# lenke182/flood-uav-video-segmentation

Hardware: AMD Instinct MI355X
Metric: segmentation FPS @713x713 (PSPNet-ResNet50 keyframe + linear interp, frame_delta=5) (higher is better)
Workload: dtype f32

## Files before the change

flood_uav_video_segmentation_amd/csrc/flow_ops.hip:

```cpp
#include "interp.h"
#include "kernels.h"

#include <type_traits>

namespace fs {

#define FS_LAUNCH_INDEXED(kernel_, total_, cap_, s_, ...)                                                                  \
    do {                                                                                                                   \
        const dim3 grid_((unsigned)std::min<int64_t>(cdiv64((total_), 256), (cap_)));                                      \
        if ((total_) < ((int64_t)1 << 31)) hipLaunchKernelGGL((kernel_<unsigned>), grid_, dim3(256), 0, (s_), __VA_ARGS__); \
        else hipLaunchKernelGGL((kernel_<int64_t>), grid_, dim3(256), 0, (s_), __VA_ARGS__);                               \
    } while (0)

template <typename I>
__global__ __launch_bounds__(256) void grid_sample_nchw_kernel(const float* __restrict__ in, int B, int C, int Hi, int Wi,
                                                               const float* __restrict__ grid, int Hg, int Wg,
                                                               float* __restrict__ out, int ac) {
    const I total = (I)B * Hg * Wg;
    for (I i = (I)blockIdx.x * 256 + threadIdx.x; i < total; i += (I)gridDim.x * 256) {
        const int b = (int)(i / ((I)Hg * Wg));
        const I g = i - (I)b * Hg * Wg;
        const float gx = grid[i * 2 + 0], gy = grid[i * 2 + 1];
        const GsTaps t = gs_taps(gx, gy, Wi, Hi, ac);
        for (int c = 0; c < C; ++c) {
// ... 46 lines not shown
        const int oy = (int)((i / Wo) % Ho);
        const I pc = i / ((I)Wo * Ho);
        const LinCoord cy = lin_coord(oy, Hi, sy, ac), cx = lin_coord(ox, Wi, sx, ac);
        out[i] = bilerp_at(in + (size_t)pc * Hi * Wi, Wi, cy, cx);
    }
}

int launch_resize_bilinear_nchw(const float* in, int BC, int Hi, int Wi, float* out, int Ho, int Wo, int align_corners,
                                hipStream_t s) {
    const int64_t total = (int64_t)BC * Ho * Wo;
    FS_LAUNCH_INDEXED(resize_bilinear_nchw_kernel, total, 16384, s, in, BC, Hi, Wi, out, Ho, Wo, align_corners,
                      resize_scale(Hi, Ho, align_corners), resize_scale(Wi, Wo, align_corners));
    FS_HIP(hipGetLastError());
    return 0;
}

template <typename I>
__global__ __launch_bounds__(256) void resize_bilinear_nhwc_kernel(const float* __restrict__ in, int ld_in, int B, int C4, int Hi,
                                                                   int Wi, float* __restrict__ out, int ld_out, int Ho, int Wo,
                                                                   int ac, float sy, float sx) {
    const I total = (I)B * Ho * Wo * C4;
    for (I i = (I)blockIdx.x * 256 + threadIdx.x; i < total; i += (I)gridDim.x * 256) {
        const int c4 = (int)(i % C4);
        const I m = i / C4;
        const int ox = (int)(m % Wo);
        const int oy = (int)((m / Wo) % Ho);
        const int b = (int)(m / ((I)Wo * Ho));
        const LinCoord cy = lin_coord(oy, Hi, sy, ac), cx = lin_coord(ox, Wi, sx, ac);
        const float* base = in + (size_t)b * Hi * Wi * ld_in + c4 * 4;
        *reinterpret_cast<f32x4*>(out + (size_t)m * ld_out + c4 * 4) = bilerp4_nhwc(base, Wi, ld_in, cy, cx);
    }
}

int launch_resize_bilinear_nhwc(const float* in, int ld_in, int B, int C, int Hi, int Wi, float* out, int ld_out, int Ho, int Wo,
                                int align_corners, hipStream_t s, int max_blocks) {
    FS_REQUIRE(C % 4 == 0 && ld_in % 4 == 0 && ld_out % 4 == 0, "resize_nhwc: C/ld must be multiples of 4");
    const int64_t total = (int64_t)B * Ho * Wo * (C / 4);
    FS_LAUNCH_INDEXED(resize_bilinear_nhwc_kernel, total, max_blocks, s, in, ld_in, B, C / 4, Hi, Wi, out, ld_out, Ho, Wo, align_corners,
                      resize_scale(Hi, Ho, align_corners), resize_scale(Wi, Wo, align_corners));
    FS_HIP(hipGetLastError());
    return 0;
}

__global__ __launch_bounds__(256) void blend_kernel(const float* __restrict__ a, float wa, const float* __restrict__ b, float wb,
                                                    float* __restrict__ out, int64_t n4, int64_t numel) {
    for (int64_t i = (int64_t)blockIdx.x * 256 + threadIdx.x; i < n4; i += (int64_t)gridDim.x * 256) {
        const f32x4 x = reinterpret_cast<const f32x4*>(a)[i];
        f32x4 r;
        if (b) {
            const f32x4 y = reinterpret_cast<const f32x4*>(b)[i];
#pragma unroll
            for (int e = 0; e < 4; ++e) r[e] = __fadd_rn(__fmul_rn(wa, x[e]), __fmul_rn(wb, y[e]));
        } else {
#pragma unroll
            for (int e = 0; e < 4; ++e) r[e] = __fmul_rn(wa, x[e]);
        }
        reinterpret_cast<f32x4*>(out)[i] = r;
    }
    if (blockIdx.x == 0) {
        for (int64_t i = n4 * 4 + threadIdx.x; i < numel; i += 256)
            out[i] = b ? __fadd_rn(__fmul_rn(wa, a[i]), __fmul_rn(wb, b[i])) : __fmul_rn(wa, a[i]);
    }
}

__global__ __launch_bounds__(256) void blend_scalar_kernel(const float* __restrict__ a, float wa, const float* __restrict__ b, float wb,
                                                           float* __restrict__ out, int64_t numel) {
    for (int64_t i = (int64_t)blockIdx.x * 256 + threadIdx.x; i < numel; i += (int64_t)gridDim.x * 256)
        out[i] = b ? __fadd_rn(__fmul_rn(wa, a[i]), __fmul_rn(wb, b[i])) : __fmul_rn(wa, a[i]);
}

int launch_blend(const float* a, float wa, const float* b, float wb, float* out, int64_t numel, hipStream_t s) {
    if ((((uintptr_t)a | (uintptr_t)b | (uintptr_t)out) & 15) != 0) {
        hipLaunchKernelGGL(blend_scalar_kernel, dim3((unsigned)std::max<int64_t>(1, std::min<int64_t>(cdiv64(numel, 256), 16384))),
                           dim3(256), 0, s, a, wa, b, wb, out, numel);
        FS_HIP(hipGetLastError());
        return 0;
    }
    const int64_t n4 = numel / 4;
    hipLaunchKernelGGL(blend_kernel, dim3((unsigned)std::max<int64_t>(1, std::min<int64_t>(cdiv64(n4, 256), 16384))), dim3(256), 0, s,
                       a, wa, b, wb, out, n4, numel);
    FS_HIP(hipGetLastError());
    return 0;
}

__device__ __forceinline__ float up_at(const float* __restrict__ pl, int h, int w, int y, int x, float sy, float sx) {
    return bilerp_at(pl, w, lin_coord(y, h, sy, 1), lin_coord(x, w, sx, 1));
}

__device__ __forceinline__ void seg_warp_step(const float* lo, const float* src, const float* grid, float* dst, int K, int h, int w, int H,
                                              int W, int Hg, int Wg, int first, float sy, float sx) {
    const int G = Hg * Wg;
    for (int g = blockIdx.x * 256 + threadIdx.x; g < G; g += gridDim.x * 256) {
        const float gx = grid[g * 2 + 0], gy = grid[g * 2 + 1];
        const int Hs = first ? H : Hg, Ws = first ? W : Wg;
        const GsTaps t = gs_taps(gx, gy, Ws, Hs, 0);
        for (int k = 0; k < K; ++k) {
            float v;
            if (first) {
                const float* pl = lo + (size_t)k * h * w;
                v = gs_sample(t, [&](int y, int x) { return up_at(pl, h, w, y, x, sy, sx); });
            } else {
                const float* pl = src + (size_t)k * G;
                v = gs_sample(t, [&](int y, int x) { return pl[y * Ws + x]; });
            }
            dst[(size_t)k * G + g] = v;
        }
    }
}

__global__ __launch_bounds__(256) void seg_warp_step_kernel(const float* __restrict__ lo_prev, const float* __restrict__ lo_next,
                                                            const float* __restrict__ src_f, const float* __restrict__ src_b,
                                                            const float* __restrict__ grid_f, const float* __restrict__ grid_b,
                                                            float* __restrict__ dst_f, float* __restrict__ dst_b, int K, int h,
                                                            int w, int H, int W, int Hg, int Wg, int first, float sy, float sx) {
    const int dir = blockIdx.y;
    seg_warp_step(dir ? lo_next : lo_prev, dir ? src_b : src_f, dir ? grid_b : grid_f, dir ? dst_b : dst_f, K, h, w, H, W, Hg, Wg, first, sy, sx);
}

template <int KMAX, bool WARP, bool CANVAS, bool DEVW>
__global__ __launch_bounds__(256) void seg_fuse_kernel(std::conditional_t<DEVW, SegTailParams, SegFuseArgs> p, float sy_lo, float sx_lo,
                                                       float sy_g, float sx_g) {
    const float* weights = nullptr;
    if constexpr (DEVW) weights = p.weights;
    const int64_t HW = (int64_t)p.H * p.W;
    const int K = p.K, n = p.n;
    const size_t cHW = (size_t)p.cH * p.cW;
    for (int y = blockIdx.y; y < p.H; y += gridDim.y) {
        const int x = blockIdx.x * 256 + threadIdx.x;
        if (x >= p.W) break;
        const int64_t i = (int64_t)y * p.W + x;
        const unsigned off4 = (unsigned)i * 4u;
        const size_t cpix = (size_t)(p.y0 + y) * p.cW + (p.x0 + x);
        float a[KMAX], b[KMAX], v[KMAX];
        auto emit = [&](int f) {
            if (p.out_logits)
#pragma unroll
                for (int k = 0; k < KMAX; ++k)
                    if (k < K) *reinterpret_cast<float*>(reinterpret_cast<char*>(p.out_logits + ((size_t)f * K + k) * HW) + off4) = v[k];
            if (p.out_mask) {
                float best = -INFINITY;
                int arg = 0;
#pragma unroll
                for (int k = 0; k < KMAX; ++k)
                    if (k < K && v[k] > best) { best = v[k]; arg = k; }
                p.out_mask[(size_t)f * HW + i] = (uint8_t)arg;
            }
            if (CANVAS) {
                softmax_k<KMAX>(v, K, [&](int k, float q) { p.canvas[((size_t)f * K + k) * cHW + cpix] += (double)q; });
                if (f == 0) p.count[cpix] += 1.0;
            }
        };
        {
            const LinCoord cy = lin_coord(y, p.h, sy_lo, 1), cx = lin_coord(x, p.w, sx_lo, 1);
#pragma unroll
            for (int k = 0; k < KMAX; ++k) {
                if (k < K) {
                    const float* pl = p.lo_prev + (size_t)k * p.h * p.w;
                    a[k] = bilerp_at(pl, p.w, cy, cx);
                    if (p.lo_next && !WARP) {
                        const float* pn = p.lo_next + (size_t)k * p.h * p.w;
                        b[k] = bilerp_at(pn, p.w, cy, cx);
                    }
                    v[k] = a[k];
                }
            }
            emit(0);
        }
        if (!p.lo_next) continue;
        LinCoord gy_c, gx_c;
        if (WARP) {
            gy_c = lin_coord(y, p.Hg, sy_g, 1);
            gx_c = lin_coord(x, p.Wg, sx_g, 1);
        }
        const int G = p.Hg * p.Wg;
        for (int f = 1; f < n; ++f) {
            const float wa = DEVW ? weights[2 * f] : (float)((double)(n - f) / (double)n);
            const float wb = DEVW ? weights[2 * f + 1] : (float)((double)f / (double)n);
            const bool hold_a = DEVW && wb == 0.f, hold_b = DEVW && !hold_a && wa == 0.f;
#pragma unroll
            for (int k = 0; k < KMAX; ++k) {
                if (k < K) {
                    float va, vb;
                    if (!WARP) {
                        va = a[k];
                        vb = b[k];
                    } else {
                        const float* pf = p.scratch + ((size_t)(f - 1) * K + k) * G;
                        const float* pb = p.scratch + ((size_t)(n - 1) * K + (size_t)(n - f - 1) * K + k) * G;
                        if (!hold_b) va = bilerp_at(pf, p.Wg, gy_c, gx_c);
                        if (!hold_a) vb = bilerp_at(pb, p.Wg, gy_c, gx_c);
                    }
                    v[k] = hold_a ? va : hold_b ? vb : __fadd_rn(__fmul_rn(wa, va), __fmul_rn(wb, vb));
                }
            }
            emit(f);
        }
    }
}

int launch_seg_tail(const SegTailParams& p, hipStream_t s) {
    FS_REQUIRE(p.K >= 1 && p.K <= 32, "seg_tail: K=%d out of range (1..32)", p.K);
    FS_REQUIRE(p.n >= 1, "seg_tail: n must be >= 1");
    FS_REQUIRE(p.out_logits || p.out_mask || p.canvas, "seg_tail: no output requested");
    FS_REQUIRE((int64_t)p.H * p.W < ((int64_t)1 << 30), "seg_tail: frames of at most 2^30 pixels");
    FS_REQUIRE(!p.canvas || (p.count && p.y0 >= 0 && p.x0 >= 0 && p.y0 + p.H <= p.cH && p.x0 + p.W <= p.cW), "seg_tail: crop outside the canvas");
    const float sy_lo = resize_scale(p.h, p.H, 1), sx_lo = resize_scale(p.w, p.W, 1);
    float sy_g = 0.f, sx_g = 0.f;
    const bool warp = p.lo_next && !p.no_warp && p.n > 1;
    if (warp) {
        FS_REQUIRE(p.scratch && p.grids_left && p.grids_right, "seg_tail: warp mode needs grids and scratch");
        sy_g = resize_scale(p.Hg, p.H, 1);
        sx_g = resize_scale(p.Wg, p.W, 1);
        const int G = p.Hg * p.Wg;
        const size_t map = (size_t)p.K * G;
        float* fwd = p.scratch;
        float* bwd = p.scratch + (size_t)(p.n - 1) * map;
        for (int j = 0; j < p.n - 1; ++j) {
            hipLaunchKernelGGL(seg_warp_step_kernel, dim3(cdiv(G, 256), 2), dim3(256), 0, s, p.lo_prev, p.lo_next,
                               j ? fwd + (size_t)(j - 1) * map : nullptr, j ? bwd + (size_t)(j - 1) * map : nullptr,
                               p.grids_left[j], p.grids_right[j], fwd + (size_t)j * map, bwd + (size_t)j * map, p.K, p.h, p.w,
                               p.H, p.W, p.Hg, p.Wg, j == 0 ? 1 : 0, sy_lo, sx_lo);
        }
    }
    const dim3 grid((unsigned)cdiv(p.W, 256), (unsigned)std::min(p.H, 65535)), block(256);
    const bool canvas = p.canvas != nullptr;
    const SegFuseArgs& a = p;
#define FS_SEG_FUSE(KM_, W_, C_)                                                                                                   \
    do {                                                                                                                           \
        if (p.weights) hipLaunchKernelGGL((seg_fuse_kernel<KM_, W_, C_, true>), grid, block, 0, s, p, sy_lo, sx_lo, sy_g, sx_g);    \
        else hipLaunchKernelGGL((seg_fuse_kernel<KM_, W_, C_, false>), grid, block, 0, s, a, sy_lo, sx_lo, sy_g, sx_g);            \
    } while (0)
    if (p.K <= 8) {
        if (warp) { if (canvas) FS_SEG_FUSE(8, true, true); else FS_SEG_FUSE(8, true, false); }
        else { if (canvas) FS_SEG_FUSE(8, false, true); else FS_SEG_FUSE(8, false, false); }
    } else {
        if (warp) { if (canvas) FS_SEG_FUSE(32, true, true); else FS_SEG_FUSE(32, true, false); }
        else { if (canvas) FS_SEG_FUSE(32, false, true); else FS_SEG_FUSE(32, false, false); }
    }
#undef FS_SEG_FUSE
    FS_HIP(hipGetLastError());
    return 0;
}

__global__ __launch_bounds__(256) void feat_warp_step_kernel(const float* __restrict__ src_f, const float* __restrict__ src_b, int Hs, int Ws,
                                                             const float* __restrict__ grid_f, const float* __restrict__ grid_b,
                                                             float* __restrict__ dst_f, float* __restrict__ dst_b, int C4, unsigned total, int S) {
    const int dir = blockIdx.y;
    const float* __restrict__ src = dir ? src_b : src_f;
    const float* __restrict__ grid = dir ? grid_b : grid_f;
    float* __restrict__ dst = dir ? dst_b : dst_f;
    const int ld = C4 * 4;
    const unsigned xcd = blockIdx.x & 7u;
    const unsigned e = (blockIdx.x >> 3) * 256u + threadIdx.x;
    const unsigned m = e / (unsigned)S;
    const int c4 = (int)(xcd * (unsigned)S + (e - m * (unsigned)S));
    if (m >= total || c4 >= C4) return;
    const float gx = grid[m * 2 + 0], gy = grid[m * 2 + 1];
    const GsTaps t = gs_taps(gx, gy, Ws, Hs, 0);
    *reinterpret_cast<f32x4*>(dst + (size_t)m * ld + c4 * 4) = gs_gather_nhwc(src + c4 * 4, Ws, ld, t);
}

struct FeatFuseArgs {
    const float* f_prev;
    const float* f_next;
    const float* chains;
    const float* grid0;
    float* stack;
    int C4, fh, fw, Hg, Wg, H0, W0, n;
    int same_g, same_0;
    float sy_g, sx_g, sy_0, sx_0;
};
struct FeatFuseWArgs : FeatFuseArgs {
    const float* weights;
};

constexpr int FEAT_RUN = 10;

struct GsCell {
    unsigned nw, ne, sw, se;
    float wnw, wne, wsw, wse;
    bool all_in;
    bool x1ok, y1ok;
};

__device__ __forceinline__ GsCell feat_cell(const FeatFuseArgs& a, int gy, int gx) {
    const size_t m = (size_t)gy * a.W0 + gx;
    const float2 g = *reinterpret_cast<const float2*>(a.grid0 + m * 2);
    const GsTaps t = gs_taps(g.x, g.y, a.fw, a.fh, 1);
    const unsigned ld = (unsigned)a.C4 * 4u;
    GsCell c;
    c.nw = (unsigned)(t.y0 * a.fw + t.x0) * ld;
    c.ne = (unsigned)(t.y0 * a.fw + t.x1) * ld;
    c.sw = (unsigned)(t.y1 * a.fw + t.x0) * ld;
    c.se = (unsigned)(t.y1 * a.fw + t.x1) * ld;
    c.wnw = t.nw; c.wne = t.ne; c.wsw = t.sw; c.wse = t.se;
    c.x1ok = t.x1ok; c.y1ok = t.y1ok;
    c.all_in = t.x1ok && t.y1ok;
    return c;
}

__device__ __forceinline__ f32x4 feat_cell_value(const float* __restrict__ cbase, const GsCell& c) {
    const f32x4 vnw = *reinterpret_cast<const f32x4*>(cbase + c.nw);
    f32x4 vne = *reinterpret_cast<const f32x4*>(cbase + c.ne);
    f32x4 vsw = *reinterpret_cast<const f32x4*>(cbase + c.sw);
    f32x4 vse = *reinterpret_cast<const f32x4*>(cbase + c.se);
    if (__builtin_amdgcn_ballot_w64(!c.all_in) != 0) {
        const f32x4 z = {0.f, 0.f, 0.f, 0.f};
        vne = c.x1ok ? vne : z;
        vsw = c.y1ok ? vsw : z;
        vse = c.all_in ? vse : z;
    }
    const f32x2 wnw = {c.wnw, c.wnw}, wne = {c.wne, c.wne}, wsw = {c.wsw, c.wsw}, wse = {c.wse, c.wse};
    f32x4 r;
    r.lo = ((vnw.lo * wnw + vne.lo * wne) + vsw.lo * wsw) + vse.lo * wse;
    r.hi = ((vnw.hi * wnw + vne.hi * wne) + vsw.hi * wsw) + vse.hi * wse;
    return r;
}

constexpr int FEAT_KEY_CH = 4;

__global__ __launch_bounds__(256) void feat_fuse_key_kernel(FeatFuseArgs a, unsigned npix, int S, int LP) {
    const int ld = a.C4 * 4;
    const unsigned xcd = blockIdx.x & 7u;
    const unsigned e = (blockIdx.x >> 3) * 256u + threadIdx.x;
    const unsigned m = e / (unsigned)LP;
    const int l = (int)(e - m * (unsigned)LP);
    if (m >= npix) return;
    const int oy = (int)(m / (unsigned)a.fw), ox = (int)(m - (unsigned)oy * (unsigned)a.fw);
    LinCoord cy, cx;
    if (a.same_0) {
        cy.i0 = cy.i1 = oy; cx.i0 = cx.i1 = ox;
        cy.w0 = cx.w0 = 1.f; cy.w1 = cx.w1 = 0.f;
    } else {
        cy = lin_coord(oy, a.H0, a.sy_0, 1);
        cx = lin_coord(ox, a.W0, a.sx_0, 1);
    }
    const GsCell c00 = feat_cell(a, cy.i0, cx.i0);
    GsCell c01 = c00, c10 = c00, c11 = c00;
    if (!a.same_0) {
        c01 = feat_cell(a, cy.i0, cx.i1);
        c10 = feat_cell(a, cy.i1, cx.i0);
        c11 = feat_cell(a, cy.i1, cx.i1);
    }
    const f32x2 wx0 = {cx.w0, cx.w0}, wx1 = {cx.w1, cx.w1}, wy0 = {cy.w0, cy.w0}, wy1 = {cy.w1, cy.w1};
#pragma unroll 1
    for (int k = 0; k < FEAT_KEY_CH; ++k) {
        const int cc = l + k * LP;
        const int c4 = (int)xcd * S + cc;
        if (cc >= S || c4 >= a.C4) break;
        const float* cbase = a.f_prev + c4 * 4;
        f32x4 r;
        if (a.same_0) {
            r = feat_cell_value(cbase, c00);
        } else {
            const f32x4 v00 = feat_cell_value(cbase, c00), v01 = feat_cell_value(cbase, c01);
            const f32x4 v10 = feat_cell_value(cbase, c10), v11 = feat_cell_value(cbase, c11);
            r.lo = wy0 * (wx0 * v00.lo + wx1 * v01.lo) + wy1 * (wx0 * v10.lo + wx1 * v11.lo);
            r.hi = wy0 * (wx0 * v00.hi + wx1 * v01.hi) + wy1 * (wx0 * v10.hi + wx1 * v11.hi);
        }
        *reinterpret_cast<f32x4*>(a.stack + (size_t)m * ld + c4 * 4) = r;
    }
}

template <bool DEVW>
__global__ __launch_bounds__(256, 6) void feat_fuse_warp_kernel(std::conditional_t<DEVW, FeatFuseWArgs, FeatFuseArgs> a, int S, int nruns) {
    const float* weights = nullptr;
    if constexpr (DEVW) weights = a.weights;
    const int ld = a.C4 * 4;
    const size_t map = (size_t)a.fh * a.fw * ld;
    const unsigned bid = blockIdx.x;
    const unsigned xcd = bid & 7u;
    const unsigned e = (bid >> 3) * 256u + threadIdx.x;
    const unsigned item = e / (unsigned)S;
    const int c4 = (int)(xcd * (unsigned)S + (e - item * (unsigned)S));
    const unsigned rowid = item / (unsigned)nruns;
    const int run = (int)(item - rowid * (unsigned)nruns);
    const int p = 1 + (int)(rowid / (unsigned)a.fh);
    const int oy = (int)(rowid - (unsigned)(p - 1) * (unsigned)a.fh);
    if (p >= a.n || c4 >= a.C4) return;
    const float wa = DEVW ? weights[2 * p] : (float)((double)(a.n - p) / (double)a.n);
    const float wb = DEVW ? weights[2 * p + 1] : (float)((double)p / (double)a.n);
    const bool hold_a = DEVW && wb == 0.f, hold_b = DEVW && !hold_a && wa == 0.f;
    const size_t cmap = (size_t)a.Hg * a.Wg * ld;
    const float* pf = a.chains + (size_t)(p - 1) * cmap + c4 * 4;
    const float* pb = a.chains + (size_t)(a.n - 1 + a.n - p - 1) * cmap + c4 * 4;
// ... 625 lines not shown
```

flood_uav_video_segmentation_amd/csrc/net_ops.hip:

```cpp
#include "interp.h"
#include "kernels.h"
#include "split.h"

#include <type_traits>

namespace fs {

template <int CPT >
__global__ __launch_bounds__(256) void stem_conv_kernel(StemParams p) {
    extern __shared__ __attribute__((aligned(16))) float wlds[];
    const int taps = p.KH * p.KW * 3;
    for (int i = threadIdx.x; i < taps * p.Cout; i += 256) wlds[i] = p.wgt[i];
    __syncthreads();

    const int groups = p.Cout / CPT;
    const int ppb = 256 / groups;
    const int cg = threadIdx.x % groups;
    const int M = p.B * p.Ho * p.Wo;
    const int m = blockIdx.x * ppb + threadIdx.x / groups;
    if (m >= M) return;
    const int hw = p.Ho * p.Wo;
    const int b = m / hw;
    const int rem = m - b * hw;
    const int oy = rem / p.Wo, ox = rem - oy * p.Wo;
// ... 256 lines not shown
        if (nsteps <= 2) FS_STEM_SPLIT_PF(NT_, 2) else FS_STEM_SPLIT_PF(NT_, 5)                                                  \
    }
        switch (p.Cout / 32) {
            case 1: FS_STEM_SPLIT(1) break;
            case 2: FS_STEM_SPLIT(2) break;
            case 3: FS_STEM_SPLIT(3) break;
            default: FS_STEM_SPLIT(4) break;
        }
#undef FS_STEM_SPLIT
#undef FS_STEM_SPLIT_PF
        FS_HIP(hipGetLastError());
        return 0;
    }
    if (p.Cout % 32 == 0 && p.Cout <= 128 && p.KH < 0x7fff) {
        const int ksteps = cdiv(cdiv(taps, 2), 8) * 8;
        const size_t lds = (size_t)2 * ksteps * (p.Cout + 2) * sizeof(float);
        FS_REQUIRE(lds <= 128 * 1024, "stem_conv: filter bank %zu B exceeds LDS budget", lds);
        FS_REQUIRE((long long)3 * (f.ncrops ? (long long)f.FH * f.FW : (long long)p.H * p.W) < (1ll << 31), "stem_conv: frame too large for 32-bit tap offsets");
        const int tiles = cdiv(M, 32);
        const dim3 grid((unsigned)std::min(cdiv(tiles, 4), 256 * 8));
#define FS_STEM_LAUNCH(NT_)                                                                                                      \
    {                                                                                                                            \
        if (lds > 64 * 1024)                                  \
            FS_HIP(hipFuncSetAttribute(reinterpret_cast<const void*>(&stem_conv_mfma_kernel<NT_>), hipFuncAttributeMaxDynamicSharedMemorySize, (int)lds)); \
        hipLaunchKernelGGL((stem_conv_mfma_kernel<NT_>), grid, dim3(256), lds, s, p, ksteps);                                    \
    }
        switch (p.Cout / 32) {
            case 1: FS_STEM_LAUNCH(1) break;
            case 2: FS_STEM_LAUNCH(2) break;
            case 3: FS_STEM_LAUNCH(3) break;
            default: FS_STEM_LAUNCH(4) break;
        }
#undef FS_STEM_LAUNCH
        FS_HIP(hipGetLastError());
        return 0;
    }
    FS_REQUIRE(256 % (p.Cout / 16) == 0, "stem_conv: the VALU kernel needs Cout / 16 to divide 256 (Cout=%d)", p.Cout);
    const int groups = p.Cout / 16, ppb = 256 / groups;
    const size_t lds = (size_t)taps * p.Cout * sizeof(float);
    FS_REQUIRE(lds <= 64 * 1024, "stem_conv: filter bank %zu B exceeds LDS budget", lds);
    hipLaunchKernelGGL((stem_conv_kernel<16>), dim3(cdiv(M, ppb)), dim3(256), lds, s, p);
    FS_HIP(hipGetLastError());
    return 0;
}

__global__ __launch_bounds__(256) void maxpool3x3s2_kernel(const float* __restrict__ in, int ld_in, float* __restrict__ out,
                                                           int ld_out, int B, int H, int W, int C4, int Ho, int Wo) {
    const unsigned r = blockIdx.x * 256 + threadIdx.x;
    if (r >= (unsigned)(Wo * C4)) return;
    const int ox = (int)(r / (unsigned)C4), c4 = (int)(r - (unsigned)ox * (unsigned)C4);
    for (int b = blockIdx.z; b < B; b += gridDim.z) {
        for (int oy = blockIdx.y; oy < Ho; oy += gridDim.y) {
            f32x4 tap[9];
#pragma unroll
            for (int ky = 0; ky < 3; ++ky) {
                const int iy = min(max(oy * 2 - 1 + ky, 0), H - 1);
#pragma unroll
                for (int kx = 0; kx < 3; ++kx) {
                    const int ix = min(max(ox * 2 - 1 + kx, 0), W - 1);
                    tap[ky * 3 + kx] = *reinterpret_cast<const f32x4*>(in + ((size_t)(b * H + iy) * W + ix) * ld_in + c4 * 4);
                }
            }
            f32x4 best = {-INFINITY, -INFINITY, -INFINITY, -INFINITY};
#pragma unroll
            for (int ky = 0; ky < 3; ++ky)
#pragma unroll
                for (int kx = 0; kx < 3; ++kx) {
                    const bool ok = (unsigned)(oy * 2 - 1 + ky) < (unsigned)H && (unsigned)(ox * 2 - 1 + kx) < (unsigned)W;
#pragma unroll
                    for (int e = 0; e < 4; ++e) best[e] = fmaxf(best[e], ok ? tap[ky * 3 + kx][e] : -INFINITY);
                }
            *reinterpret_cast<f32x4*>(out + ((size_t)(b * Ho + oy) * Wo + ox) * ld_out + c4 * 4) = best;
        }
    }
}

int launch_maxpool3x3s2(const float* in, int ld_in, float* out, int ld_out, int B, int H, int W, int C, int Ho, int Wo,
                        hipStream_t s) {
    FS_REQUIRE(C % 4 == 0 && ld_in % 4 == 0 && ld_out % 4 == 0, "maxpool: C/ld must be multiples of 4");
    FS_REQUIRE((int64_t)Wo * (C / 4) < (int64_t)1 << 31, "maxpool: output row too large");
    hipLaunchKernelGGL(maxpool3x3s2_kernel, dim3((unsigned)cdiv(Wo * (C / 4), 256), (unsigned)std::min(Ho, 65535), (unsigned)std::min(B, 65535)), dim3(256), 0, s,
                       in, ld_in, out, ld_out, B, H, W, C / 4, Ho, Wo);
    FS_HIP(hipGetLastError());
    return 0;
}

__global__ __launch_bounds__(256) void adaptive_avgpool_kernel(const float* __restrict__ in, int ld_in, float* __restrict__ out,
                                                               int H, int W, int C, int bin) {
    __shared__ f32x4 part[32][8];
    const int cell = blockIdx.x, b = blockIdx.z;
    const int by = cell / bin, bx = cell - by * bin;
    const int ys = (by * H) / bin, ye = ((by + 1) * H + bin - 1) / bin;
    const int xs = (bx * W) / bin, xe = ((bx + 1) * W + bin - 1) / bin;
    const int wh = ye - ys, ww = xe - xs;
    const int cl = threadIdx.x & 7, pg = threadIdx.x >> 3;
    const int c = blockIdx.y * 32 + cl * 4;
    f32x4 acc = {0.f, 0.f, 0.f, 0.f};
    for (int i = pg; i < wh * ww; i += 32) {
        const int y = ys + i / ww, x = xs + i % ww;
        const f32x4 v = *reinterpret_cast<const f32x4*>(in + ((size_t)(b * H + y) * W + x) * ld_in + c);
        acc += v;
    }
    part[pg][cl] = acc;
    __syncthreads();
    if (pg == 0) {
        f32x4 sum = part[0][cl];
        for (int g = 1; g < 32; ++g) sum += part[g][cl];
        const float inv = 1.f / (float)(wh * ww);
        sum *= inv;
        *reinterpret_cast<f32x4*>(out + ((size_t)b * bin * bin + cell) * C + c) = sum;
    }
}

int launch_adaptive_avgpool(const float* in, int ld_in, float* out, int B, int H, int W, int C, int bin, hipStream_t s) {
    FS_REQUIRE(C % 32 == 0 && ld_in % 4 == 0, "adaptive_avgpool: C=%d must be a multiple of 32", C);
    hipLaunchKernelGGL(adaptive_avgpool_kernel, dim3(bin * bin, C / 32, B), dim3(256), 0, s, in, ld_in, out, H, W, C, bin);
    FS_HIP(hipGetLastError());
    return 0;
}

__global__ __launch_bounds__(256) void ppm_pool_combine_kernel(const float* __restrict__ cell_mean , float* __restrict__ out1,
                                                               float* __restrict__ out2, float* __restrict__ out3, int B, int C) {
    const int64_t total = (int64_t)B * C;
    for (int64_t i = (int64_t)blockIdx.x * 256 + threadIdx.x; i < total; i += (int64_t)gridDim.x * 256) {
        const int c = (int)(i % C), b = (int)(i / C);
        const float* m = cell_mean + (size_t)b * 36 * C + c;
        float s3[9], s2[4] = {0.f, 0.f, 0.f, 0.f}, s1 = 0.f;
#pragma unroll
        for (int k = 0; k < 9; ++k) s3[k] = 0.f;
#pragma unroll
        for (int y = 0; y < 6; ++y)
#pragma unroll
            for (int x = 0; x < 6; ++x) {
                const float v = m[(size_t)(y * 6 + x) * C];
                s3[(y / 2) * 3 + x / 2] += v;
                s2[(y / 3) * 2 + x / 3] += v;
                s1 += v;
            }
#pragma unroll
        for (int k = 0; k < 9; ++k) out3[((size_t)b * 9 + k) * C + c] = s3[k] * 0.25f;
#pragma unroll
        for (int k = 0; k < 4; ++k) out2[((size_t)b * 4 + k) * C + c] = s2[k] * (1.f / 9.f);
        out1[(size_t)b * C + c] = s1 * (1.f / 36.f);
    }
}

int launch_ppm_pool_combine(const float* cell_mean, float* out1, float* out2, float* out3, int B, int C, hipStream_t s) {
    const int64_t total = (int64_t)B * C;
    hipLaunchKernelGGL(ppm_pool_combine_kernel, dim3((unsigned)cdiv64(total, 256)), dim3(256), 0, s, cell_mean, out1, out2, out3, B, C);
    FS_HIP(hipGetLastError());
    return 0;
}

template <int KV >
__global__ __launch_bounds__(256) void rowdot_1x1_kernel(RowdotBatch pb, int ld_in, int ld_out, int K, int N, int relu) {
    const RowdotProblem& q = pb.p[blockIdx.z];
    const int lane = threadIdx.x & 63;
    const int n = blockIdx.x * 4 + (threadIdx.x >> 6);
    if (n >= N) return;
    const int M = q.M;
    const int per = (M + gridDim.y - 1) / gridDim.y;
    const int m_begin = blockIdx.y * per, m_end = min(M, (int)(blockIdx.y + 1) * per);
    if (m_begin >= m_end) return;
    f32x4 w[KV];
#pragma unroll
    for (int i = 0; i < KV; ++i) w[i] = *reinterpret_cast<const f32x4*>(q.wgt + (size_t)n * K + (i * 64 + lane) * 4);
    const float sc = q.scale ? q.scale[n] : 1.f, sh = q.shift ? q.shift[n] : 0.f;
    for (int m = m_begin; m < m_end; ++m) {
        float acc = 0.f;
#pragma unroll
        for (int i = 0; i < KV; ++i) {
            const f32x4 x = *reinterpret_cast<const f32x4*>(q.in + (size_t)m * ld_in + (i * 64 + lane) * 4);
            acc += x[0] * w[i][0] + x[1] * w[i][1] + x[2] * w[i][2] + x[3] * w[i][3];
        }
#pragma unroll
        for (int off = 32; off > 0; off >>= 1) acc += __shfl_xor(acc, off, 64);
        if (lane == 0) {
            float y = acc * sc + sh;
            if (relu) y = fmaxf(y, 0.f);
            q.out[(size_t)m * ld_out + n] = y;
        }
    }
}

int launch_rowdot_1x1_batch(const RowdotBatch& pb, int nprob, int ld_in, int ld_out, int K, int N, int relu, hipStream_t s) {
    FS_REQUIRE(K % 256 == 0 && K <= 4096, "rowdot_1x1: K=%d must be a multiple of 256 and <= 4096", K);
    FS_REQUIRE(nprob >= 1 && nprob <= 4, "rowdot_1x1: 1..4 problems per launch");
    int mmax = 1;
    for (int i = 0; i < nprob; ++i) mmax = std::max(mmax, pb.p[i].M);
    const dim3 grid(cdiv(N, 4), std::max(1, std::min(12, mmax / 6)), nprob), block(256);
#define FS_ROWDOT(KV)                                                                                             \
    case KV:                                                                                                      \
        hipLaunchKernelGGL((rowdot_1x1_kernel<KV>), grid, block, 0, s, pb, ld_in, ld_out, K, N, relu);            \
        break;
    switch (K / 256) {
        FS_ROWDOT(1) FS_ROWDOT(2) FS_ROWDOT(3) FS_ROWDOT(4) FS_ROWDOT(5) FS_ROWDOT(6) FS_ROWDOT(7) FS_ROWDOT(8)
        FS_ROWDOT(9) FS_ROWDOT(10) FS_ROWDOT(11) FS_ROWDOT(12) FS_ROWDOT(13) FS_ROWDOT(14) FS_ROWDOT(15) FS_ROWDOT(16)
        default: return fail("rowdot_1x1: unsupported K");
    }
#undef FS_ROWDOT
    FS_HIP(hipGetLastError());
    return 0;
}

int launch_rowdot_1x1(const float* in, int ld_in, const float* wgt, const float* scale, const float* shift, float* out,
                      int ld_out, int M, int K, int N, int relu, hipStream_t s) {
    RowdotBatch pb{};
    pb.p[0] = RowdotProblem{in, wgt, scale, shift, out, M};
    return launch_rowdot_1x1_batch(pb, 1, ld_in, ld_out, K, N, relu, s);
}

int launch_upsample_into(const float* in, int hi, int wi, float* out, int ld_out, int B, int Ho, int Wo, int C,
                         int align_corners, hipStream_t s) {
    FS_REQUIRE(C % 4 == 0 && ld_out % 4 == 0 && ((uintptr_t)out & 15) == 0, "upsample_into: C/ld_out must be multiples of 4");
    return launch_resize_bilinear_nhwc(in, C, B, C, hi, wi, out, ld_out, Ho, Wo, align_corners, s, 256 * 32);
}

__global__ __launch_bounds__(256) void classifier_nchw_kernel(const float* __restrict__ in, int ld_in, const float* __restrict__ wgt,
                                                              const float* __restrict__ bias, float* __restrict__ out, int B,
                                                              int HW, int C, int K) {
    extern __shared__ __attribute__((aligned(16))) float wl[];
    for (int i = threadIdx.x; i < K * C; i += 256) wl[i] = wgt[i];
    __syncthreads();
    const int l16 = threadIdx.x & 15;
    const int64_t M = (int64_t)B * HW;
    const int64_t m = (int64_t)blockIdx.x * 16 + (threadIdx.x >> 4);
    const int64_t mc = m < M ? m : M - 1;
    const float* x = in + (size_t)mc * ld_in;
    for (int k0 = 0; k0 < K; k0 += 8) {
        float acc[8];
#pragma unroll
        for (int k = 0; k < 8; ++k) acc[k] = 0.f;
        for (int c = l16 * 4; c < C; c += 64) {
            const f32x4 v = *reinterpret_cast<const f32x4*>(x + c);
#pragma unroll
            for (int k = 0; k < 8; ++k) {
                if (k0 + k < K) {
                    const f32x4 w = *reinterpret_cast<const f32x4*>(wl + (size_t)(k0 + k) * C + c);
                    acc[k] += v[0] * w[0] + v[1] * w[1] + v[2] * w[2] + v[3] * w[3];
                }
            }
        }
#pragma unroll
        for (int k = 0; k < 8; ++k) {
#pragma unroll
            for (int off = 8; off > 0; off >>= 1) acc[k] += __shfl_xor(acc[k], off, 64);
        }
        if (l16 == 0 && m < M) {
            const int64_t b = m / HW, pix = m - b * HW;
#pragma unroll
            for (int k = 0; k < 8; ++k)
                if (k0 + k < K) out[((size_t)b * K + k0 + k) * HW + pix] = acc[k] + (bias ? bias[k0 + k] : 0.f);
        }
    }
}

int launch_classifier_nchw(const float* in, int ld_in, const float* wgt, const float* bias, float* out, int B, int HW,
                           int C, int K, hipStream_t s) {
    FS_REQUIRE(C % 4 == 0 && ld_in % 4 == 0, "classifier: C must be a multiple of 4");
    const size_t lds = (size_t)K * C * sizeof(float);
    FS_REQUIRE(lds <= 64 * 1024, "classifier: K*C too large for LDS");
    const int64_t M = (int64_t)B * HW;
    hipLaunchKernelGGL(classifier_nchw_kernel, dim3((unsigned)cdiv64(M, 16)), dim3(256), lds, s, in, ld_in, wgt, bias, out, B,
                       HW, C, K);
    FS_HIP(hipGetLastError());
    return 0;
}

__global__ void pack_weights_kernel(const float* __restrict__ w, float* __restrict__ out, int O, int I, int KH, int KW, int hwio) {
    const int64_t total = (int64_t)O * I * KH * KW;
    for (int64_t i = (int64_t)blockIdx.x * blockDim.x + threadIdx.x; i < total; i += (int64_t)gridDim.x * blockDim.x) {
        const int s = (int)(i % KW);
        const int r = (int)((i / KW) % KH);
        const int ci = (int)((i / ((int64_t)KW * KH)) % I);
        const int o = (int)(i / ((int64_t)KW * KH * I));
        size_t dst;
        if (hwio == 1)
            dst = ((size_t)((r * KW + s) * I + ci)) * O + o;
        else if (hwio == 2)
            dst = (((size_t)o * (I / 32) + ci / 32) * KH * KW + r * KW + s) * 32 + (ci & 31);
        else
            dst = ((size_t)((o * KH + r) * KW + s)) * I + ci;
        out[dst] = w[i];
    }
}

int launch_pack_oihw_to_ohwi(const float* w, float* out, int O, int I, int KH, int KW, hipStream_t s) {
    const int64_t total = (int64_t)O * I * KH * KW;
    hipLaunchKernelGGL(pack_weights_kernel, dim3((unsigned)std::min<int64_t>(cdiv64(total, 256), 65535)), dim3(256), 0, s, w, out,
                       O, I, KH, KW, 0);
    FS_HIP(hipGetLastError());
    return 0;
}
int launch_pack_oihw_chunk_major(const float* w, float* out, int O, int I, int KH, int KW, hipStream_t s) {
    FS_REQUIRE(I % 32 == 0, "pack(chunk-major): Cin must be a multiple of 32");
    const int64_t total = (int64_t)O * I * KH * KW;
    hipLaunchKernelGGL(pack_weights_kernel, dim3((unsigned)std::min<int64_t>(cdiv64(total, 256), 65535)), dim3(256), 0, s, w, out,
                       O, I, KH, KW, 2);
    FS_HIP(hipGetLastError());
    return 0;
}
int launch_pack_oihw_to_hwio(const float* w, float* out, int O, int I, int KH, int KW, hipStream_t s) {
    const int64_t total = (int64_t)O * I * KH * KW;
    hipLaunchKernelGGL(pack_weights_kernel, dim3((unsigned)std::min<int64_t>(cdiv64(total, 256), 65535)), dim3(256), 0, s, w, out,
                       O, I, KH, KW, 1);
    FS_HIP(hipGetLastError());
    return 0;
}

__global__ __launch_bounds__(256) void concat_scaled_filters_kernel(const float* __restrict__ wa, const float* __restrict__ sa,
                                                                    const float* __restrict__ ha, int Ka, const float* __restrict__ wb,
                                                                    const float* __restrict__ sb, const float* __restrict__ hb, int Kb,
                                                                    float* __restrict__ out, float* __restrict__ shift_out, int O) {
    const int K = Ka + Kb;
    const int64_t total = (int64_t)O * K;
    for (int64_t i = (int64_t)blockIdx.x * 256 + threadIdx.x; i < total; i += (int64_t)gridDim.x * 256) {
        const int k = (int)(i % K), o = (int)(i / K);
        out[i] = k < Ka ? sa[o] * wa[(size_t)o * Ka + k] : sb[o] * wb[(size_t)o * Kb + (k - Ka)];
        if (k == 0) shift_out[o] = ha[o] + hb[o];
    }
}
int launch_concat_scaled_filters(const float* wa, const float* sa, const float* ha, int Ka, const float* wb, const float* sb, const float* hb,
                                 int Kb, float* out, float* shift_out, int O, hipStream_t s) {
    FS_REQUIRE(wa && sa && ha && wb && sb && hb && out && shift_out && O >= 1 && Ka >= 1 && Kb >= 1, "concat_scaled_filters: bad arguments");
    const int64_t total = (int64_t)O * (Ka + Kb);
    hipLaunchKernelGGL(concat_scaled_filters_kernel, dim3((unsigned)std::min<int64_t>(cdiv64(total, 256), 65535)), dim3(256), 0, s, wa, sa, ha, Ka,
                       wb, sb, hb, Kb, out, shift_out, O);
    FS_HIP(hipGetLastError());
    return 0;
}

__global__ __launch_bounds__(256) void pack_slice_tap_major_kernel(const float* __restrict__ w, float* __restrict__ out, int O, int I,
                                                                   int c0, int nc, int taps) {
    const int64_t total = (int64_t)taps * O * nc;
    for (int64_t i = (int64_t)blockIdx.x * 256 + threadIdx.x; i < total; i += (int64_t)gridDim.x * 256) {
        const int c = (int)(i % nc);
        const int o = (int)((i / nc) % O);
        const int tap = (int)(i / ((int64_t)nc * O));
        out[i] = w[((size_t)o * I + c0 + c) * taps + tap];
    }
}
int launch_pack_slice_tap_major(const float* w, float* out, int O, int I, int c0, int nc, int taps, hipStream_t s) {
    FS_REQUIRE(c0 >= 0 && nc >= 1 && c0 + nc <= I, "pack(slice): channel range outside the filter bank");
// ... 219 lines not shown
```

Measured before the change: 1261.

## Register-block rowdot over rows and channels; specialize seg fuse for K=5

The 1x1 rowdot kernel now has each wavefront compute several output channels for several input rows at once. Input rows and weight vectors are kept in registers and reused, the shuffle reductions are batched, and the grid is reshaped to match. Separately, the segmentation fuse kernel gets a K=5 non-warp, non-canvas instantiation that gathers all four bilinear taps for every class before interpolating. Both changes aim to raise load-level parallelism and cut redundant global loads, at the cost of higher register pressure and some clamped duplicate loads at the edges.

```diff
diff --git a/flood_uav_video_segmentation_amd/csrc/flow_ops.hip b/flood_uav_video_segmentation_amd/csrc/flow_ops.hip
--- a/flood_uav_video_segmentation_amd/csrc/flow_ops.hip
+++ b/flood_uav_video_segmentation_amd/csrc/flow_ops.hip
@@ -222,6 +222,30 @@
         };
         {
             const LinCoord cy = lin_coord(y, p.h, sy_lo, 1), cx = lin_coord(x, p.w, sx_lo, 1);
+            if constexpr (KMAX <= 8 && !CANVAS) {
+                const int o00 = cy.i0 * p.w + cx.i0, o01 = cy.i0 * p.w + cx.i1, o10 = cy.i1 * p.w + cx.i0, o11 = cy.i1 * p.w + cx.i1;
+                const size_t plane = (size_t)p.h * p.w;
+                const bool both = p.lo_next && !WARP;
+                float ta[KMAX][4], tb[KMAX][4];
+#pragma unroll
+                for (int k = 0; k < KMAX; ++k) {
+                    const float* pl = p.lo_prev + (size_t)min(k, K - 1) * plane;
+                    ta[k][0] = pl[o00]; ta[k][1] = pl[o01]; ta[k][2] = pl[o10]; ta[k][3] = pl[o11];
+                }
+                if (both) {
+#pragma unroll
+                    for (int k = 0; k < KMAX; ++k) {
+                        const float* pn = p.lo_next + (size_t)min(k, K - 1) * plane;
+                        tb[k][0] = pn[o00]; tb[k][1] = pn[o01]; tb[k][2] = pn[o10]; tb[k][3] = pn[o11];
+                    }
+                }
+#pragma unroll
+                for (int k = 0; k < KMAX; ++k) {
+                    a[k] = bilerp(ta[k][0], ta[k][1], ta[k][2], ta[k][3], cy, cx);
+                    if (both) b[k] = bilerp(tb[k][0], tb[k][1], tb[k][2], tb[k][3], cy, cx);
+                    v[k] = a[k];
+                }
+            } else
 #pragma unroll
             for (int k = 0; k < KMAX; ++k) {
                 if (k < K) {
@@ -300,7 +324,9 @@
         if (p.weights) hipLaunchKernelGGL((seg_fuse_kernel<KM_, W_, C_, true>), grid, block, 0, s, p, sy_lo, sx_lo, sy_g, sx_g);    \
         else hipLaunchKernelGGL((seg_fuse_kernel<KM_, W_, C_, false>), grid, block, 0, s, a, sy_lo, sx_lo, sy_g, sx_g);            \
     } while (0)
-    if (p.K <= 8) {
+    if (p.K == 5 && !warp && !canvas) {
+        FS_SEG_FUSE(5, false, false);
+    } else if (p.K <= 8) {
         if (warp) { if (canvas) FS_SEG_FUSE(8, true, true); else FS_SEG_FUSE(8, true, false); }
         else { if (canvas) FS_SEG_FUSE(8, false, true); else FS_SEG_FUSE(8, false, false); }
     } else {
diff --git a/flood_uav_video_segmentation_amd/csrc/net_ops.hip b/flood_uav_video_segmentation_amd/csrc/net_ops.hip
--- a/flood_uav_video_segmentation_amd/csrc/net_ops.hip
+++ b/flood_uav_video_segmentation_amd/csrc/net_ops.hip
@@ -432,34 +432,68 @@
     return 0;
 }
 
+constexpr int rowdot_rows(int KV) { return KV <= 8 ? 4 : 2; }
+constexpr int rowdot_chans(int KV) { return KV <= 8 ? 4 : 2; }
+
 template <int KV >
 __global__ __launch_bounds__(256) void rowdot_1x1_kernel(RowdotBatch pb, int ld_in, int ld_out, int K, int N, int relu) {
+    constexpr int R = rowdot_rows(KV), NW = rowdot_chans(KV);
     const RowdotProblem& q = pb.p[blockIdx.z];
     const int lane = threadIdx.x & 63;
-    const int n = blockIdx.x * 4 + (threadIdx.x >> 6);
-    if (n >= N) return;
+    const int n0 = (blockIdx.x * 4 + (threadIdx.x >> 6)) * NW;
+    if (n0 >= N) return;
     const int M = q.M;
-    const int per = (M + gridDim.y - 1) / gridDim.y;
+    const int per = ((M + gridDim.y - 1) / gridDim.y + R - 1) / R * R;
     const int m_begin = blockIdx.y * per, m_end = min(M, (int)(blockIdx.y + 1) * per);
     if (m_begin >= m_end) return;
-    f32x4 w[KV];
-#pragma unroll
-    for (int i = 0; i < KV; ++i) w[i] = *reinterpret_cast<const f32x4*>(q.wgt + (size_t)n * K + (i * 64 + lane) * 4);
+    auto load_w = [&](int j, f32x4 (&w)[KV]) {
+        const float* wr = q.wgt + (size_t)min(n0 + j, N - 1) * K + lane * 4;
+#pragma unroll
+        for (int i = 0; i < KV; ++i) w[i] = *reinterpret_cast<const f32x4*>(wr + i * 256);
+    };
+    const int oj = (lane / R) % NW, orow = lane % R;
+    const int n = min(n0 + oj, N - 1);
     const float sc = q.scale ? q.scale[n] : 1.f, sh = q.shift ? q.shift[n] : 0.f;
-    for (int m = m_begin; m < m_end; ++m) {
-        float acc = 0.f;
-#pragma unroll
-        for (int i = 0; i < KV; ++i) {
-            const f32x4 x = *reinterpret_cast<const f32x4*>(q.in + (size_t)m * ld_in + (i * 64 + lane) * 4);
-            acc += x[0] * w[i][0] + x[1] * w[i][1] + x[2] * w[i][2] + x[3] * w[i][3];
-        }
-#pragma unroll
-        for (int off = 32; off > 0; off >>= 1) acc += __shfl_xor(acc, off, 64);
-        if (lane == 0) {
-            float y = acc * sc + sh;
-            if (relu) y = fmaxf(y, 0.f);
-            q.out[(size_t)m * ld_out + n] = y;
-        }
+    for (int m0 = m_begin; m0 < m_end; m0 += R) {
+        constexpr int WB = KV <= 8 ? 2 : 1;
+        f32x4 x[R][KV], w[WB][KV];
+#pragma unroll
+        for (int r = 0; r < R; ++r) {
+            const float* xr = q.in + (size_t)min(m0 + r, m_end - 1) * ld_in + lane * 4;
+#pragma unroll
+            for (int i = 0; i < KV; ++i) x[r][i] = *reinterpret_cast<const f32x4*>(xr + i * 256);
+        }
+        load_w(0, w[0]);
+        float acc[NW][R];
+#pragma unroll
+        for (int j = 0; j < NW; ++j) {
+            if (WB == 2 && j + 1 < NW) load_w(j + 1, w[(j + 1) % WB]);
+            if (WB == 1 && j > 0) load_w(j, w[0]);
+#pragma unroll
+            for (int r = 0; r < R; ++r) {
+                float a = 0.f;
+#pragma unroll
+                for (int i = 0; i < KV; ++i) {
+                    const f32x4 xv = x[r][i], wv = w[j % WB][i];
+                    a += xv[0] * wv[0] + xv[1] * wv[1] + xv[2] * wv[2] + xv[3] * wv[3];
+                }
+                acc[j][r] = a;
+            }
+        }
+#pragma unroll
+        for (int off = 32; off > 0; off >>= 1)
+#pragma unroll
+            for (int j = 0; j < NW; ++j)
+#pragma unroll
+                for (int r = 0; r < R; ++r) acc[j][r] += __shfl_xor(acc[j][r], off, 64);
+        float v = acc[0][0];
+#pragma unroll
+        for (int j = 0; j < NW; ++j)
+#pragma unroll
+            for (int r = 0; r < R; ++r) v = (oj == j && orow == r) ? acc[j][r] : v;
+        float y = v * sc + sh;
+        if (relu) y = fmaxf(y, 0.f);
+        if (lane < NW * R && m0 + orow < m_end && n0 + oj < N) q.out[(size_t)(m0 + orow) * ld_out + n] = y;
     }
 }
 
@@ -468,7 +502,8 @@
     FS_REQUIRE(nprob >= 1 && nprob <= 4, "rowdot_1x1: 1..4 problems per launch");
     int mmax = 1;
     for (int i = 0; i < nprob; ++i) mmax = std::max(mmax, pb.p[i].M);
-    const dim3 grid(cdiv(N, 4), std::max(1, std::min(12, mmax / 6)), nprob), block(256);
+    const int KV = K / 256, R = rowdot_rows(KV), NW = rowdot_chans(KV);
+    const dim3 grid(cdiv(N, 4 * NW), std::min(32, cdiv(mmax, R)), nprob), block(256);
 #define FS_ROWDOT(KV)                                                                                             \
     case KV:                                                                                                      \
         hipLaunchKernelGGL((rowdot_1x1_kernel<KV>), grid, block, 0, s, pb, ld_in, ld_out, K, N, relu);            \
```

Result: no change. 1260, median of 3 (-0.0%).
